# shaunplee/ray-tracing

Hardware: AMD Instinct MI355X
Metric: Msamples/s (WxHxspp/s) + achieved HBM GB/s, final scene 1200x800x500spp (higher is better)
Workload: dtype f64

## Files before the change

include/rt_wide.h:

```cpp
#pragma once
#include <stdint.h>

#define RT_WIDE 4

typedef struct rt_wnode {
  float lo[3][RT_WIDE];
  float hi[3][RT_WIDE];
  int32_t child[RT_WIDE];
  int32_t pad[RT_WIDE];
} rt_wnode;

typedef struct rt_qnode {
  float origin[3];
  float scale[3];
  uint32_t qlo[3];
  uint32_t qhi[3];
  int32_t child[RT_WIDE];
} rt_qnode;

#define RT_WKEY_BITS 14
#define RT_WKEY_MASK ((1u << RT_WKEY_BITS) - 1u)
#define RT_WKEY_MAX_IDS (1 << (RT_WKEY_BITS - 1))
#define RT_WKEY_REJECTED 0x7f800000u

#if defined(__HIPCC__) || defined(__CUDACC__)
#define RT_WKEY_FN __host__ __device__ static inline
#else
#define RT_WKEY_FN static inline
#endif

RT_WKEY_FN int rt_wkey_fits(long long n_wide_nodes, long long n_leaf_slots) {
  return n_wide_nodes <= RT_WKEY_MAX_IDS && n_leaf_slots <= RT_WKEY_MAX_IDS;
}
RT_WKEY_FN int32_t rt_wkey_pack(uint32_t key_bits, int32_t ref) {
  return (int32_t)((key_bits & ~RT_WKEY_MASK) | ((uint32_t)ref & RT_WKEY_MASK));
}
RT_WKEY_FN int32_t rt_wkey_ref(int32_t word) {
  const uint32_t low = (uint32_t)word & RT_WKEY_MASK;
  return (int32_t)(low ^ (1u << (RT_WKEY_BITS - 1))) - (1 << (RT_WKEY_BITS - 1));
}

RT_WKEY_FN int rt_wkey_beyond(int32_t word, float tmax32, float slack) {
  const uint32_t kb = (uint32_t)word & ~RT_WKEY_MASK;
  float key;
  __builtin_memcpy(&key, &kb, sizeof key);
  return key * (1.0f - 0x1p-21f) > __builtin_fmaf(tmax32, 1.0f + 0x1p-21f, slack);
}

#ifdef __cplusplus
static_assert(sizeof(rt_wnode) == 128, "rt_wnode is 128 bytes");
static_assert(sizeof(rt_qnode) == 64, "rt_qnode is 64 bytes");
#endif
```

ray-tracing_amd/csrc/rt_kernels.h:

```cpp
#pragma once
#include <hip/hip_runtime.h>

#include <algorithm>
#include <cstdlib>
#include <cmath>
#include <cstdio>
#include <cstring>
#include <string>
#include <vector>

#include "rt.h"
#include "rt_device.h"
#include "rt_error.h"
#include "rt_internal.h"
#include "rt_trace.h"

using namespace rtd;

namespace {

struct UDiv {
  uint32_t m;
  int s1, s2;
};
// ... 259 lines not shown
        } else {
          w = -1;
        }
      }
    }
    if (w < 0) break;
    if (!path) {
      const uint32_t pid = (uint32_t)((long long)row * L.W + px);
      g.init(A.seed, pid, (uint32_t)s);
      g.reserve(3);
      const double ru = g.draw(), rv = g.draw();
      const int y = L.H - 1 - row;
      const double u = ((double)px + ru) / (double)L.W;
      const double v = ((double)y + rv) / (double)L.H;
      ray = get_ray(L.cam, u, v, g);
      thr = v3(1.0, 1.0, 1.0);
      depth = L.max_depth;
      path = true;
    }
    V3 contrib;
    if constexpr ((F & F_COUNT) != 0) {
      segs += depth > 0;
      s1 = stamp();
      s2 = s1;
    }
    bool ended = segment<F>(A, S, L.S, ray, thr, depth, g, stk, contrib, cnt, stride, &s2);
    if (!ended && thr.x != thr.x && thr.y != thr.y && thr.z != thr.z) {
      contrib = vmul(thr, v3(0.0, 0.0, 0.0));
      ended = true;
    }
    if constexpr ((F & F_COUNT) != 0) {
      const unsigned long long s3 = stamp();
      ph_acq += s1 - s0;
      ph_trav += s2 - s1;
      ph_shade += s3 - s2;
    }
    if (ended) {
      if constexpr ((F & F_COUNT) != 0) {
        blocks += g.pair;
        ++samples;
      }
      if (A.flags & RT_FLAG_NAN_ZERO) contrib = nan_zero(contrib);
      sum = sum + contrib;
      path = false;
      ++s;
      const bool all_nan = (A.flags & RT_FLAG_NAN_CULL) && sum.x != sum.x && sum.y != sum.y && sum.z != sum.z;
      if (s == s_end || all_nan) {
        store_partial(L, w, sum);
        w = -1;
      }
    }
  }
  if constexpr ((F & F_COUNT) != 0) {
    wave_add(&L.work[0], segs);
    wave_add(&L.work[1], cnt.box);
    wave_add(&L.work[2], cnt.prim);
    wave_add(&L.work[3], cnt.other);
    wave_add(&L.work[4], cnt.light);
    wave_add(&L.work[5], blocks);
    wave_add(&L.work[6], samples);
    if ((threadIdx.x & 63) == 0) {
      atomicAdd(&L.work[8], ph_acq);
      atomicAdd(&L.work[9], ph_trav);
      atomicAdd(&L.work[10], ph_shade);
    }
  }
}

template <unsigned F, int WAVES>
__global__ void __launch_bounds__(RT_BLOCK, WAVES) render_philox(RenderArgs A) {
  __shared__ __attribute__((aligned(16))) int stk_mem[kLcBytes / 4 + RT_STACK * RT_BLOCK];
  const LaunchConst& L = stage_const(A, stk_mem);
  __syncthreads();
  philox_loop<F>(A, L, A.S, &stk_mem[kLcBytes / 4 + threadIdx.x], RT_BLOCK);
}

template <unsigned F, int WAVES>
__global__ void __launch_bounds__(WAVES * 256, WAVES) render_philox_lds(RenderArgs A, int n_nodes, int stack_entries) {
  extern __shared__ __attribute__((aligned(16))) unsigned char lds[];
  const LaunchConst& L = stage_const(A, lds);
  rt_node* nodes = reinterpret_cast<rt_node*>(lds + kLcBytes);
  {
    const uint4* src = reinterpret_cast<const uint4*>(A.S.nodes);
    uint4* dst = reinterpret_cast<uint4*>(lds + kLcBytes);
    const int n16 = n_nodes * (int)(sizeof(rt_node) / 16);
    for (int i = threadIdx.x; i < n16; i += blockDim.x) dst[i] = src[i];
  }
  __syncthreads();
  Scene S = A.S;
  S.nodes = nodes;
  int* stk = reinterpret_cast<int*>(lds + kLcBytes + (size_t)n_nodes * sizeof(rt_node)) + threadIdx.x;
  (void)stack_entries;
  philox_loop<F>(A, L, S, stk, WAVES * 256);
}


template <unsigned F, bool PK = false>
__device__ __forceinline__ void philox_loop2(const RenderArgs& A, const LaunchConst& L, const Scene& S, int* stk,
                                             int stride, int* side_p, volatile uint32_t* wq) {
  const int lane = threadIdx.x & 63;
  const unsigned long long lanes_below = (lane == 0) ? 0ull : (~0ull >> (64 - lane));
  const bool joint = !(A.flags & RT_FLAG_REFERENCE_CULL);

  long long w = -1;
  bool done = false, walking = false, ready = false;
  if (lane == 0) {
    wq[0] = 0u;
    wq[1] = 0u;
  }
  constexpr int kLoop = (F & F_WIDE) ? 2 : 1;
  constexpr bool kLaneLds = lane_lds_of(F, kLoop);
  int l_px = 0, l_row = 0, l_s_end = 0, l_depth = 0;
  int* ex = side_p + side_ints_of(F, S.frames, kLoop) * stride;
  int& px = kLaneLds ? ex[0] : l_px;
  int& row = kLaneLds ? ex[stride] : l_row;
  int& s_end = kLaneLds ? ex[2 * stride] : l_s_end;
  int& depth = kLaneLds ? ex[3 * stride] : l_depth;
  px = 0, row = 0, s_end = 0, depth = 0;
  int s = 0;
  V3 thr = v3(0, 0, 0), sum = v3(0, 0, 0);
  RngPhilox g;
  g.init(A.seed, 0, 0);
  Trav t;
  Side side{side_p, stride, S.frames};
  Cnt cnt{};
  if constexpr ((F & F_COUNT) != 0) cnt.prof = A.prof;
  unsigned long long segs = 0, blocks = 0, samples = 0, ph_setup = 0, ph_trav = 0, ph_shade = 0;

  auto end_sample = [&](V3 contrib) __attribute__((always_inline)) {
    if constexpr ((F & F_COUNT) != 0) {
      blocks += g.pair;
      ++samples;
    }
    if (A.flags & RT_FLAG_NAN_ZERO) contrib = nan_zero(contrib);
    const V3 sm = sum + contrib;
    sum = sm;
    ++s;
    const bool all_nan = (A.flags & RT_FLAG_NAN_CULL) && sm.x != sm.x && sm.y != sm.y && sm.z != sm.z;
    if (s == s_end || all_nan) {
      if (kTail<F> && w >= kTailSlot) store_partial_at(L.tail_buf, w - kTailSlot, contrib);
      else store_partial(L, w, sm);
      w = -1;
    }
  };
  auto all_nan3 = [](const V3& a) __attribute__((always_inline)) { return a.x != a.x && a.y != a.y && a.z != a.z; };

  for (;;) {
    unsigned long long s0 = 0;
    if constexpr ((F & F_COUNT) != 0) {
      s0 = stamp();
      ++cnt.oslot;
    }
    if (ready && (t.tie || (kRefMixed<F> && t.lite)) && !t.redo) {
      ready = false;
      if constexpr ((F & F_COUNT) != 0) ++cnt.ties;
      trav_redo<F>(t, L.S.world_ref, INFINITY);
      if constexpr ((F & F_WIDE) != 0) t.ray = prep(plain(t.ray));
      walking = true;
    }
    bool start = false;
    if (ready) {
      ready = false;
      Hit h;
      Ray ray = plain(t.ray);
      const bool got = trav_finish<F>(L.S, t, ray, kEps, h, side);
      V3 contrib;
      V3 th = thr;
      if (shade_hit<F>(L.S, got, h, ray, th, depth, g, contrib, cnt)) {
        end_sample(contrib);
      } else if (depth <= 0 || all_nan3(th)) {
        end_sample(vmul(th, v3(0.0, 0.0, 0.0)));
      } else {
        thr = th;
        t.ray.o = ray.o;
        t.ray.d = ray.d;
        t.ray.tm = ray.tm;
        start = true;
        if constexpr ((F & F_COUNT) != 0) ++segs;
      }
    }
    unsigned long long s0b = 0;
    if constexpr ((F & F_COUNT) != 0) s0b = stamp();
    while (!walking && !start) {
      for (;;) {
        const bool need = (w < 0) && !done;
        const unsigned long long mask = __ballot(need);
        if (!mask) break;
        const uint32_t n_need = (uint32_t)__popcll(mask);
        const uint32_t q_next = wq[0], q_end = wq[1];
        const uint32_t avail = q_end - q_next;
        uint32_t base2 = q_next, end2 = q_end;
        if (avail < n_need) {
          const int leader = __ffsll((long long)mask) - 1;
          unsigned long long claim = 0;
          if (lane == leader) {
            const uint32_t want = n_need - avail;
            const long long rem = L.work_total - (long long)q_end;
            const uint32_t b = rem <= 0 ? 0u : max((uint32_t)L.batch_floor,
                                                   (uint32_t)fminf((float)L.batch, (float)rem * L.batch_per_item));
            const uint32_t got = want < b ? b : want;
            const unsigned long long c0 = atomicAdd(L.counter, (unsigned long long)got);
            claim = (c0 < 0xffff0000ull ? c0 : 0xffff0000ull) | ((unsigned long long)got << 32);
          }
          const unsigned long long c1 = __shfl(claim, leader);
          base2 = (uint32_t)c1;
          end2 = base2 + (uint32_t)(c1 >> 32);
        }
        const uint32_t rank = (uint32_t)__popcll(mask & lanes_below);
        if (need) {
          const long long wi = (long long)(rank < avail ? q_next + rank : base2 + (rank - avail));
          if (wi >= L.work_total) {
            done = true;
          } else if (kTail<F> ? work_unit<(F & F_SKIP) != 0>(L, (uint32_t)wi, px, row, s, s_end, w)
                              : work_item<(F & F_SKIP) != 0>(L, (uint32_t)wi, px, row, s, s_end, w)) {
            sum = v3(0, 0, 0);
          } else {
            w = -1;
          }
        }
        const int leader = __ffsll((long long)mask) - 1;
        if (lane == leader) {
          wq[0] = avail < n_need ? base2 + (n_need - avail) : q_next + n_need;
          wq[1] = end2;
        }
      }
      if (w < 0) break;
      const uint32_t pid = (uint32_t)((long long)row * L.W + px);
      g.init(A.seed, pid, (uint32_t)s);
      g.reserve(3);
      const double ru = g.draw(), rv = g.draw();
      const int y = L.H - 1 - row;
      const double u = ((double)px + ru) / (double)L.W;
      const double v = ((double)y + rv) / (double)L.H;
      const Ray cray = get_ray(L.cam, u, v, g);
      t.ray.o = cray.o;
      t.ray.d = cray.d;
      t.ray.tm = cray.tm;
      thr = v3(1.0, 1.0, 1.0);
      depth = L.max_depth;
      if (depth <= 0) {
        end_sample(vmul(v3(1.0, 1.0, 1.0), v3(0.0, 0.0, 0.0)));
        continue;
      }
      start = true;
      if constexpr ((F & F_COUNT) != 0) ++segs;
    }
    if (start) {
      trav_begin<F>(t, plain(t.ray), S.world, kEps, INFINITY);
      if (S.ref_walk) trav_restart_ref(t, S.world, INFINITY);
      trav_media_first<F>(S, t, kEps, cnt, g, side);
      walking = true;
    }
    if (!walking) break;
    unsigned long long s1 = 0;
    if constexpr ((F & F_COUNT) != 0) s1 = stamp();
    const int live = __popcll(__ballot(true));
    const int stop = (live * A.trav_stop) >> 6;
    const int ls = (F & F_WIDE) ? A.leaf_stop : A.box_first;
    walk_until<F, PK>(S, t, walking, kEps, stk, stride, joint, stop, (live * ls) >> 6, cnt, g, side, A.med_batch);
    ready = !walking;
    if constexpr ((F & F_COUNT) != 0) {
      const unsigned long long s2 = stamp();
      ph_shade += s0b - s0;
      ph_setup += s1 - s0b;
      ph_trav += s2 - s1;
    }
  }
  if constexpr ((F & F_COUNT) != 0) {
    wave_add(&L.work[0], segs);
    wave_add(&L.work[1], cnt.box);
    wave_add(&L.work[2], cnt.prim);
    wave_add(&L.work[3], cnt.other);
    wave_add(&L.work[4], cnt.light);
    wave_add(&L.work[5], blocks);
    wave_add(&L.work[6], samples);
    wave_add(&L.work[7], cnt.wide);
    wave_add(&L.work[11], cnt.islot);
    wave_add(&L.work[12], cnt.lslot);
    wave_add(&L.work[13], cnt.oslot);
    wave_add(&L.work[14], cnt.phit);
    wave_add(&L.work[15], cnt.ties);
    if ((threadIdx.x & 63) == 0) {
      atomicAdd(&L.work[8], ph_setup);
      atomicAdd(&L.work[9], ph_trav);
      atomicAdd(&L.work[10], ph_shade);
    }
  }
}

template <unsigned F>
constexpr int lane_ints() {
  return ((F & (F_WIDE | F_MIXW)) ? RT_WSTACK : RT_STACK) + ((F & F_FRAMES) ? kSideInts : 0);
}

template <unsigned F, int WAVES>
__global__ void __launch_bounds__(RT_BLOCK, WAVES) render_philox2(RenderArgs A, int stack_entries) {
  extern __shared__ __attribute__((aligned(16))) int stk_mem[];
  __shared__ uint32_t wave_q[RT_BLOCK / 64][2];
  const LaunchConst& L = stage_const(A, stk_mem);
  __syncthreads();
  int* lane0 = &stk_mem[kLcBytes / 4 + threadIdx.x];
  philox_loop2<F>(A, L, A.S, lane0, RT_BLOCK, lane0 + stack_entries * RT_BLOCK,
                  wave_q[__builtin_amdgcn_readfirstlane(threadIdx.x >> 6)]);
}

template <unsigned F>
__global__ void __launch_bounds__(RT_BLOCK, 1) render_philox2_count_packed(RenderArgs A, int stack_entries) {
  static_assert((F & F_WIDE) != 0 && (F & F_COUNT) != 0, "the 4-wide counting build only");
  extern __shared__ __attribute__((aligned(16))) int stk_mem[];
  __shared__ uint32_t wave_q[RT_BLOCK / 64][2];
  const LaunchConst& L = stage_const(A, stk_mem);
// ... 757 lines not shown
```

ray-tracing_amd/csrc/rt_trace.h:

```cpp
#pragma once
#include "rt_device.h"

namespace rtd {

template <unsigned F>
constexpr bool kRay32 = (F & (F_WIDE | F_MIXW)) != 0;
template <unsigned F>
constexpr bool kNoInv = (F & F_WIDE) != 0 && (F & (F_ALL | F_MIXW)) == 0;

struct Cnt {
  unsigned box, prim, other, light, wide;
  unsigned islot, lslot, oslot;
  unsigned phit;
  unsigned ties;
  unsigned long long* prof;
};
enum : unsigned { K_BOX = 1u, K_WIDE = 2u, K_LEAF = 4u, K_MEDIUM = 8u, K_FRAME = 16u };

__device__ __forceinline__ int hmod256(long long a) {
  const long long r = a % 256;
  return (int)(r < 0 ? r + 256 : r);
}
__device__ inline double noise(const rt_perlin* P, double sc, V3 p) {
  const V3 q = scale(sc, p);
// ... 804 lines not shown
  }
  if constexpr ((F & F_MEDIA) != 0) {
    const Ray r = plain(t.ray);
    const double rec1tp = gmax(t_min, t1);
    const double rec2t = R::kKeyed ? tt : gmin(t.closest, tt);
    if (rec1tp >= rec2t) return;
    const double rec1t = rec1tp < 0 ? 0 : rec1tp;
    const double ray_length = vlen(r.d);
    const double dist_inside = (rec2t - rec1t) * ray_length;
    double rnd;
    if constexpr (R::kKeyed) rnd = g.keyed(medium_key(n));
    else rnd = g.draw();
    const double hit_dist = n->f[0] * log_call(rnd);
    if (hit_dist > dist_inside) return;
    const double x = rec1t + (hit_dist / ray_length);
    if constexpr (R::kKeyed) {
      if (!(x <= t.closest)) return;
      trav_take<F>(S, t, x, id, kSubMedium, side, refsem, n, false);
    } else {
      trav_take<F>(S, t, x, id, kSubMedium, side, true, n, false);
    }
  }
}

typedef float f32x2 __attribute__((ext_vector_type(2)));

__device__ __forceinline__ void wide_keys2(const Trav& t, f32x2 nx, f32x2 ny, f32x2 nz, f32x2 fx, f32x2 fy, f32x2 fz,
                                           float& k0, float& k1) {
  const f32x2 ox = {t.o32x, t.o32x}, oy = {t.o32y, t.o32y}, oz = {t.o32z, t.o32z};
  const f32x2 ix = {t.i32x, t.i32x}, iy = {t.i32y, t.i32y}, iz = {t.i32z, t.i32z};
  const f32x2 tnx = (nx - ox) * ix, tny = (ny - oy) * iy, tnz = (nz - oz) * iz;
  const f32x2 tfx = (fx - ox) * ix, tfy = (fy - oy) * iy, tfz = (fz - oz) * iz;
  const float n0 = fmaxf(fmaxf(tnx.x, tny.x), fmaxf(tnz.x, t.tmin32));
  const float n1 = fmaxf(fmaxf(tnx.y, tny.y), fmaxf(tnz.y, t.tmin32));
  const float f0 = fminf(fminf(tfx.x, tfy.x), fminf(tfz.x, t.tmax32));
  const float f1 = fminf(fminf(tfx.y, tfy.y), fminf(tfz.y, t.tmax32));
  const bool h0 = n0 * (1.0f - 0x1p-21f) <= fmaf(f0, 1.0f + 0x1p-21f, t.slack);
  const bool h1 = n1 * (1.0f - 0x1p-21f) <= fmaf(f1, 1.0f + 0x1p-21f, t.slack);
  k0 = h0 ? fminf(n0, 3.0e38f) : INFINITY;
  k1 = h1 ? fminf(n1, 3.0e38f) : INFINITY;
}

__device__ __forceinline__ void cswap(float& ka, int& ca, float& kb, int& cb) {
  const bool s = kb < ka;
  const float k = s ? kb : ka;
  const int c = s ? cb : ca;
  kb = s ? ka : kb;
  cb = s ? ca : cb;
  ka = k;
  ca = c;
}

__device__ __forceinline__ void pswap(int& a, int& b) {
  const int lo = min(a, b);
  b = max(a, b);
  a = lo;
}

__device__ __forceinline__ float4 qplanes(uint32_t q, float s, float o) {
  return float4{fmaf((float)(q & 255u), s, o), fmaf((float)((q >> 8) & 255u), s, o),
                fmaf((float)((q >> 16) & 255u), s, o), fmaf((float)(q >> 24), s, o)};
}

template <unsigned F = 0, bool PK = false>
__device__ __forceinline__ bool wide_node(const Scene& S, Trav& t, int* stk, int stride, int w) {
  float4 nx, ny, nz, fx, fy, fz;
  int4 ch;
  if constexpr ((F & F_QNODE) != 0) {
    const uint4* qb = reinterpret_cast<const uint4*>(&S.qnodes[w]);
    const uint4 a = qb[0], b = qb[1], c = qb[2];
    const uint4 d = qb[3];
    ch = int4{(int)d.x, (int)d.y, (int)d.z, (int)d.w};
    const float ox = __uint_as_float(a.x), oy = __uint_as_float(a.y), oz = __uint_as_float(a.z);
    const float sx = __uint_as_float(a.w), sy = __uint_as_float(b.x), sz = __uint_as_float(b.y);
    const bool mx = signbit(t.i32x), my = signbit(t.i32y), mz = signbit(t.i32z);
    nx = qplanes(mx ? c.y : b.z, sx, ox);
    fx = qplanes(mx ? b.z : c.y, sx, ox);
    ny = qplanes(my ? c.z : b.w, sy, oy);
    fy = qplanes(my ? b.w : c.z, sy, oy);
    nz = qplanes(mz ? c.w : c.x, sz, oz);
    fz = qplanes(mz ? c.x : c.w, sz, oz);
  } else {
    const float* base = reinterpret_cast<const float*>(&S.wnodes[w]);
    const int ox = signbit(t.i32x) ? 12 : 0, oy = signbit(t.i32y) ? 16 : 4, oz = signbit(t.i32z) ? 20 : 8;
    nx = *reinterpret_cast<const float4*>(base + ox);
    ny = *reinterpret_cast<const float4*>(base + oy);
    nz = *reinterpret_cast<const float4*>(base + oz);
    fx = *reinterpret_cast<const float4*>(base + (ox ^ 12));
    fy = *reinterpret_cast<const float4*>(base + (oy < 12 ? oy + 12 : oy - 12));
    fz = *reinterpret_cast<const float4*>(base + (oz < 12 ? oz + 12 : oz - 12));
    ch = *reinterpret_cast<const int4*>(base + 24);
  }
  float k0, k1, k2, k3;
  wide_keys2(t, f32x2{nx.x, nx.y}, f32x2{ny.x, ny.y}, f32x2{nz.x, nz.y}, f32x2{fx.x, fx.y}, f32x2{fy.x, fy.y},
             f32x2{fz.x, fz.y}, k0, k1);
  wide_keys2(t, f32x2{nx.z, nx.w}, f32x2{ny.z, ny.w}, f32x2{nz.z, nz.w}, f32x2{fx.z, fx.w}, f32x2{fy.z, fy.w},
             f32x2{fz.z, fz.w}, k2, k3);
  int c0 = ch.x, c1 = ch.y, c2 = ch.z, c3 = ch.w;
  const int n_hit = (k0 < INFINITY) + (k1 < INFINITY) + (k2 < INFINITY) + (k3 < INFINITY);
  if constexpr (PK) {
    int p0 = rt_wkey_pack(__float_as_uint(k0), c0), p1 = rt_wkey_pack(__float_as_uint(k1), c1);
    int p2 = rt_wkey_pack(__float_as_uint(k2), c2), p3 = rt_wkey_pack(__float_as_uint(k3), c3);
    pswap(p0, p1);
    pswap(p2, p3);
    pswap(p0, p2);
    pswap(p1, p3);
    pswap(p1, p2);
    c0 = rt_wkey_ref(p0);
    c1 = p1;
    c2 = p2;
    c3 = p3;
  } else {
    cswap(k0, c0, k1, c1);
    cswap(k2, c2, k3, c3);
    cswap(k0, c0, k2, c2);
    cswap(k1, c1, k3, c3);
    cswap(k1, c1, k2, c2);
  }
  const int e0 = n_hit > 3 ? c3 : (n_hit > 2 ? c2 : c1);
  const int e1 = n_hit > 3 ? c2 : c1;
  stk[t.sp * stride] = e0;
  stk[(t.sp + 1) * stride] = e1;
  stk[(t.sp + 2) * stride] = c1;
  t.sp += n_hit > 1 ? n_hit - 1 : 0;
  t.node = c0;
  return n_hit != 0;
}

constexpr int kNone = (int)0x80000000;

template <unsigned F>
__device__ __forceinline__ bool trav_pop_mixed(const Scene& S, Trav& t, const int* stk, int stride, Side& side,
                                               double t_min = kEps) {
  bool reb = false;
  for (;;) {
    const bool end = t.sp == 0;
    const int e = end ? 0 : stk[(--t.sp) * stride];
    const bool frame = (F & F_FRAMES) && ((F & F_MIXW) ? (e >= 0 && (e & RT_FRAME)) : (e & RT_FRAME));
    if (end || !frame) {
      if ((F & F_FRAMES) && reb) {
        Ray pr = side.get_ray();
        for (int k = 0; k < t.level; ++k) pr = enter_instance(&S.nodes[side.frame(k)], pr);
        t.ray = prep(pr);
        if constexpr ((F & F_MIXW) != 0) set_ray32(t, t_min);
      }
      t.node = e;
      return !end;
    }
    --t.level;
    reb = true;
  }
}

template <unsigned F, class R>
__device__ __forceinline__ bool trav_step(const Scene& S, Trav& t, double t_min, int* stk, int stride, bool joint,
                                          Cnt& cnt, R& g, Side& side) {
  bool wide = false;
  if constexpr ((F & F_WIDE) != 0) wide = !t.ref;
  if (wide) {
    if (t.node >= 0) {
      if constexpr ((F & F_COUNT) != 0) ++cnt.wide;
      if (wide_node<F>(S, t, stk, stride, t.node)) return true;
    } else {
      const rt_node* n = &S.leaves[~t.node];
      trav_leaf<F>(S, t, n, ~t.node | kSlotTag, t_min, cnt, g, side, false);
    }
    if (t.sp == 0) return false;
    t.node = stk[(--t.sp) * stride];
    return true;
  }
  bool leaf_slot = false, to_wide = false;
  if constexpr ((F & F_MIXW) != 0) {
    to_wide = t.node >= 0 && (t.node & RT_WNODE);
    leaf_slot = t.node < 0;
  }
  if (!to_wide) {
  int id = leaf_slot ? (~(t.node | RT_ISMED) | kSlotTag) : (t.node & ~(RT_SUB | RT_IDTAGS));
  int tag = leaf_slot ? RT_SUB : (kRefMixed<F> ? (t.node & RT_SUB) : 0);
  bool refsem = t.ref && !tag;
  const rt_node* n = leaf_slot ? &S.leaves[~(t.node | RT_ISMED)] : &S.nodes[id];
  const int tf = n->type;
  const int type = tf & RT_TYPE_MASK;
  if (type == RT_NODE_BVH) {
   constexpr int kFuse = (F & F_WIDE) ? 0 : 8;
   for (int fuse = 0;; ++fuse) {
    if (fuse) {
      id = t.node & ~(RT_SUB | RT_IDTAGS);
      tag = kRefMixed<F> ? (t.node & RT_SUB) : 0;
      refsem = t.ref && !tag;
      n = &S.nodes[id];
    }
    const bool same = kRefMixed<F> && (t.node & RT_IDTAGS) == RT_SAMEBOX;
    if constexpr ((F & F_COUNT) != 0) cnt.box += !same;
    if (same || box_hit(n->f, t.ray, t_min, refsem ? t.closest : closest_up<F>(t), joint)) {
      const int c = n->c;
      const bool ord = (c & RT_BVH_ORDERED) && !t.redo;
      if constexpr ((F & F_MIXW) != 0) {
        if (ord && (c & RT_WROOT)) {
          t.node = RT_WNODE | ((c >> 2) & RT_WROOT_MASK);
          to_wide = true;
          break;
        }
      }
      const bool flip = ord && !(c & RT_BVH_MEDIA_FIRST) && comp(t.ray.d, c & 3) < 0;
      const int ctag = (kRefMixed<F> && ord) ? RT_SUB : tag;
      stk[(t.sp++) * stride] = (flip ? n->a : n->b) | ctag;
      t.node = (flip ? n->b : n->a) | ctag;
      if ((t.node & RT_ISBOX) && fuse < kFuse) continue;
      return true;
    }
    break;
   }
  } else if ((F & F_FRAMES) && (type == RT_NODE_TRANSLATE || type == RT_NODE_ROTATE) && !(tf & RT_CHAIN_PRIM)) {
    if (t.level == 0) side.put_ray(plain(t.ray));
    Ray cr = plain(t.ray);
    int cur = leaf_slot ? n->c : id, ct = tf;
    if ((F & F_MIXW) && leaf_slot && (tf & RT_FRAME_FUSED)) {
      rt_node rec;
      {
        const uint4* q = reinterpret_cast<const uint4*>(n);
        const uint4 q0 = q[0], q1 = q[1], q2 = q[2], q3 = q[3];
        uint4* r = reinterpret_cast<uint4*>(&rec);
        r[0] = q0, r[1] = q1, r[2] = q2, r[3] = q3;
      }
      cur = rec.c;
      if constexpr ((F & F_COUNT) != 0) ++cnt.other;
      side.frame(t.level++) = cur;
      stk[(t.sp++) * stride] = RT_FRAME | cur;
      cr = enter_instance(&rec, cr);
      if (tf & RT_FRAME_FUSED2) {
        if constexpr ((F & F_COUNT) != 0) ++cnt.other;
        side.frame(t.level++) = rec.a;
        stk[(t.sp++) * stride] = RT_FRAME | rec.a;
        const int ax = (tf >> RT_FRAME_AX2_SHIFT) & 3;
        cr = Ray{unrotate_point(ax, rec.f[3], rec.f[4], cr.o), unrotate_point(ax, rec.f[3], rec.f[4], cr.d), cr.tm};
      }
      const int inner = (int)rec.f[5];
      t.ray = prep(cr);
      set_ray32(t, t_min);
      t.node = (inner & RT_WNODE) ? inner : (inner | tag);
      return true;
    } else {
      do {
        if constexpr ((F & F_COUNT) != 0) ++cnt.other;
        side.frame(t.level++) = cur;
        stk[(t.sp++) * stride] = RT_FRAME | cur;
        cr = enter_instance(&S.nodes[cur], cr);
        cur = S.nodes[cur].a;
        ct = S.nodes[cur].type;
      } while (((ct & RT_TYPE_MASK) == RT_NODE_TRANSLATE || (ct & RT_TYPE_MASK) == RT_NODE_ROTATE) &&
               !(ct & RT_CHAIN_PRIM));
    }
    t.ray = prep(cr);
    if constexpr ((F & F_MIXW) != 0) set_ray32(t, t_min);
    t.node = cur | tag;
    return true;
  } else {
    trav_leaf<F>(S, t, n, id, t_min, cnt, g, side, refsem);
  }
  if (!to_wide) return trav_pop_mixed<F>(S, t, stk, stride, side, t_min);
  }
  if constexpr ((F & F_MIXW) != 0) {
    if constexpr ((F & F_COUNT) != 0) ++cnt.wide;
    refresh_ray32(t);
    if (wide_node<F>(S, t, stk, stride, t.node & ~RT_WNODE)) return true;
  }
  return trav_pop_mixed<F>(S, t, stk, stride, side, kEps);
}


template <bool PK = false>
__device__ __forceinline__ int trav_pop(Trav& t, const int* stk, int stride) {
  if constexpr (PK) {
    return t.sp ? rt_wkey_ref(stk[(--t.sp) * stride]) : kNone;
  } else {
    return t.sp ? stk[(--t.sp) * stride] : kNone;
  }
}
template <bool PK = false>
__device__ __forceinline__ void trav_postpone(Trav& t, int* stk, int stride) {
  if (t.node < 0 && t.node != kNone && t.pend < 0) {
    t.pend = ~t.node;
    t.node = trav_pop<PK>(t, stk, stride);
  }
}
template <unsigned F, bool PK = false>
__device__ __forceinline__ void wide_inner(const Scene& S, Trav& t, int* stk, int stride, Cnt& cnt) {
  if constexpr ((F & F_COUNT) != 0) ++cnt.wide;
  if (!wide_node<F, PK>(S, t, stk, stride, t.node)) t.node = trav_pop<PK>(t, stk, stride);
  trav_postpone<PK>(t, stk, stride);
}
template <unsigned F, bool PK = false, class R>
__device__ __forceinline__ void wide_leaf(const Scene& S, Trav& t, double t_min, int* stk, int stride, Cnt& cnt, R& g,
                                          Side& side) {
  for (int k = 0; k < 1 && t.pend >= 0; ++k) {
    const rt_node* n = &S.leaves[t.pend];
    [[maybe_unused]] const float bound_before = t.tmax32;
    trav_leaf<F>(S, t, n, t.pend | kSlotTag, t_min, cnt, g, side, false);
    t.pend = -1;
    if constexpr (PK && (F & F_RECT) == 0) {
      if (t.tmax32 < bound_before)
        while (t.sp && rt_wkey_beyond(stk[(t.sp - 1) * stride], t.tmax32, t.slack)) --t.sp;
    }
  }
  trav_postpone<PK>(t, stk, stride);
}

template <unsigned F, bool PK = false, class R>
__device__ __forceinline__ void walk_until(const Scene& S, Trav& t, bool& walking, double t_min, int* stk, int stride,
                                           bool joint, int stop, int leaf_stop, Cnt& cnt, R& g, Side& side,
                                           int med_batch = 0) {
  if constexpr ((F & F_WIDE) == 0) {
    for (;;) {
      const int n_walk = __popcll(__ballot(walking));
      if (n_walk <= stop) break;
      constexpr bool kBoxFirst = kRefMixed<F>;
      const bool box_id = walking && t.node >= 0 && (t.node & (RT_ISBOX | RT_WNODE));
      const bool at_box = kBoxFirst && box_id;
      int ty = -1;
      if constexpr ((F & F_COUNT) != 0) {
        if (walking) {
          if ((F & F_MIXW) && t.node < 0) ty = S.leaves[~(t.node | RT_ISMED)].type & RT_TYPE_MASK;
          else if (box_id) ty = RT_NODE_BVH;
          else ty = S.nodes[t.node & ~(RT_SUB | RT_IDTAGS)].type & RT_TYPE_MASK;
        }
      }
      bool go = walking;
      if constexpr (kBoxFirst) {
        const int n_box = __popcll(__ballot(at_box));
        if (leaf_stop < n_walk && n_box > leaf_stop) {
          go = walking && at_box;
        } else if ((F & F_MEDIA) && med_batch > 0) {
          const bool at_med = walking && t.node >= 0 && (t.node & (RT_WNODE | RT_IDTAGS)) == RT_ISMED;
          const int n_med = __popcll(__ballot(at_med));
          if (n_med < med_batch && n_med < n_walk) go = walking && !at_med;
        }
      }
      if constexpr ((F & F_COUNT) != 0) {
        ++cnt.islot;
        const bool inst = ty == RT_NODE_TRANSLATE || ty == RT_NODE_ROTATE;
        const bool box = ty == RT_NODE_BVH;
        cnt.lslot += (__ballot(go && box) != 0) + (__ballot(go && inst) != 0) +
                     (__ballot(go && ty == RT_NODE_CONSTANT_MEDIUM) != 0) +
                     (__ballot(go && !box && !inst && ty != RT_NODE_CONSTANT_MEDIUM) != 0);
      }
      unsigned kinds = 0;
      unsigned long long t0 = 0;
      if constexpr ((F & F_COUNT) != 0) {
        const bool wide = walking && t.node >= 0 && (t.node & RT_WNODE);
        const bool inst = ty == RT_NODE_TRANSLATE || ty == RT_NODE_ROTATE;
        bool frame = false;
        if (inst) {
          const int nid = t.node < 0 ? -1 : (t.node & ~(RT_SUB | RT_IDTAGS));
          const int tf = t.node < 0 ? S.leaves[~(t.node | RT_ISMED)].type : S.nodes[nid].type;
          frame = !(tf & RT_CHAIN_PRIM);
        }
        kinds = (__ballot(go && ty == RT_NODE_BVH && !wide) ? K_BOX : 0u) | (__ballot(go && wide) ? K_WIDE : 0u) |
                (__ballot(go && ty == RT_NODE_CONSTANT_MEDIUM) ? K_MEDIUM : 0u) | (__ballot(go && frame) ? K_FRAME : 0u) |
                (__ballot(go && ty >= 0 && ty != RT_NODE_BVH && ty != RT_NODE_CONSTANT_MEDIUM && !frame) ? K_LEAF : 0u);
        t0 = stamp();
      }
      if (go) walking = trav_step<F>(S, t, t_min, stk, stride, joint, cnt, g, side);
      if constexpr ((F & F_COUNT) != 0) {
        const unsigned long long t1 = stamp();
        if (cnt.prof && __lane_id() == (unsigned)(__ffsll((long long)__ballot(true)) - 1)) {
          atomicAdd(&cnt.prof[kinds], t1 - t0);
          atomicAdd(&cnt.prof[32 + kinds], 1ull);
        }
      }
    }
  } else {
    for (;;) {
      if (__popcll(__ballot(walking)) <= stop) break;
      const bool seeking = walking && (t.ref || (t.pend < 0 && t.node >= 0));
      const bool holding = walking && !t.ref && t.pend >= 0;
      unsigned kinds = 0;
      unsigned long long t0 = 0;
      if constexpr ((F & F_COUNT) != 0) t0 = stamp();
      if (__popcll(__ballot(seeking)) > leaf_stop || __ballot(holding) == 0) {
        if constexpr ((F & F_COUNT) != 0) {
          ++cnt.islot;
          kinds = __ballot(walking && t.ref) ? K_BOX | K_WIDE : K_WIDE;
        }
        if (walking && t.ref) {
          walking = trav_step<F>(S, t, t_min, stk, stride, joint, cnt, g, side);
        } else if (walking && t.node >= 0) {
          wide_inner<F, PK>(S, t, stk, stride, cnt);
          walking = t.node != kNone || t.pend >= 0;
        }
      } else {
        if constexpr ((F & F_COUNT) != 0) {
          ++cnt.lslot;
          kinds = K_LEAF;
        }
        if (holding) {
          wide_leaf<F, PK>(S, t, t_min, stk, stride, cnt, g, side);
          walking = t.node != kNone || t.pend >= 0;
        }
      }
      if constexpr ((F & F_COUNT) != 0) {
        const unsigned long long t1 = stamp();
        if (cnt.prof && __lane_id() == (unsigned)(__ffsll((long long)__ballot(true)) - 1)) {
          atomicAdd(&cnt.prof[kinds], t1 - t0);
          atomicAdd(&cnt.prof[32 + kinds], 1ull);
        }
      }
    }
  }
}

template <unsigned F>
__device__ __forceinline__ bool trav_finish(const Scene& S, const Trav& t, const Ray& r, double t_min, Hit& h,
                                            const Side& side) {
  if (t.best_node < 0) return false;
  const bool slot = (F & (F_WIDE | F_MIXW)) && (t.best_node & kSlotTag);
  const rt_node* n = slot ? &S.leaves[t.best_node & ~kSlotTag] : &S.nodes[t.best_node];
  int levels = 0;
  if constexpr ((F & F_FRAMES) != 0) levels = t.best_level;
  Ray fr = r;
  int sub = t.best_sub;
  const rt_node* leaf = n;
  int chain_id = -1, chain_len = 0;
  if constexpr ((F & F_FRAMES) != 0)
    for (int k = 0; k < levels; ++k) fr = enter_instance(&S.nodes[side.best(k)], fr);
  bool med = false;
  if constexpr ((F & F_MEDIA) != 0) med = sub == kSubMedium;
  if (med) {
    h.t = t.closest;
    h.p = at(fr, t.closest);
    h.n = v3(1, 0, 0);
    h.u = 0;
    h.v = 0;
    h.ff = 1;
    h.mat = n->b;
  }
  if constexpr ((F & F_INST) != 0) {
    if (!med && (sub & kSubChain)) {
      sub &= ~kSubChain;
      chain_id = slot ? n->c : t.best_node;
      int cur = chain_id;
      while ((S.nodes[cur].type & RT_TYPE_MASK) == RT_NODE_TRANSLATE || (S.nodes[cur].type & RT_TYPE_MASK) == RT_NODE_ROTATE) {
        fr = enter_instance(&S.nodes[cur], fr);
        cur = S.nodes[cur].a;
        ++chain_len;
      }
      leaf = &S.nodes[cur];
    }
  }
  if (!med) prim_record<F>(S, leaf, sub, fr, t.closest, h);
  for (int lv = levels + chain_len - 1; lv >= 0; --lv) {
    Ray rl = r;
    const rt_node* inst = nullptr;
    int cur = chain_id;
    for (int k = 0; k <= lv; ++k) {
      if ((F & F_FRAMES) && k < levels) {
        inst = &S.nodes[side.best(k)];
      } else {
        inst = &S.nodes[cur];
        cur = inst->a;
      }
      rl = enter_instance(inst, rl);
    }
    exit_instance(inst, rl, h);
  }
  return true;
}

template <unsigned F, int D>
__device__ __forceinline__ double htbl_pdf_value(const Scene& S, int id, V3 origin, V3 v, const RayX& r) {
  id &= ~RT_IDTAGS;
  const rt_node* n = &S.nodes[id];
  const int type = n->type & RT_TYPE_MASK;
  Hit hh;
  if (type == RT_NODE_RECT_XZ) {
    if (!rect_hit(1, n->f[0], n->f[1], n->f[2], n->f[3], n->f[4], n->a, r, kEps, INFINITY, hh)) return 0.0;
    const double area = (n->f[1] - n->f[0]) * (n->f[3] - n->f[2]);
    const double distance_squared = hh.t * hh.t * sqlen(v);
    const double cosine = fabs(dot(v, hh.n) / vlen(v));
    return distance_squared / (cosine * area);
  }
  if (type == RT_NODE_SPHERE) {
    double t;
    if (!sphere_t(vload(n->f), n->f[3], r, kEps, INFINITY, t)) return 0.0;
    const double radius = n->f[3];
    const double cos_theta_max = sqrt(1 - radius * radius / sqlen(vload(n->f) - origin));
    const double solid_angle = 2 * kPi * (1 - cos_theta_max);
    return 1 / solid_angle;
  }
  if constexpr (D > 0) {
    if (type == RT_NODE_BVH) {
      if (!box_hit(n->f, r, kEps, INFINITY, false)) return 0.0;
      const double left_pdf = htbl_pdf_value<F, D - 1>(S, n->a, origin, v, r) + 0;
      const double left_w = (double)S.nodes[n->a & ~RT_IDTAGS].c / (double)n->c;
      const double right_pdf = htbl_pdf_value<F, D - 1>(S, n->b, origin, v, r) + 0;
      const double right_w = (double)S.nodes[n->b & ~RT_IDTAGS].c / (double)n->c;
      return left_w * left_pdf + right_w * right_pdf;
    }
  }
  return 0.0;
}

template <class R>
__device__ inline V3 htbl_random(const Scene& S, int id, V3 o, R& g) {
  if (id >= 0) id &= ~RT_IDTAGS;
  while (id >= 0 && (S.nodes[id].type & RT_TYPE_MASK) == RT_NODE_BVH) {
    const rt_node* n = &S.nodes[id];
    const double rd = g.draw();
    id = (rd < (double)S.nodes[n->a & ~RT_IDTAGS].c / (double)n->c ? n->a : n->b) & ~RT_IDTAGS;
  }
  if (id < 0) return v3(1, 0, 0);
  const rt_node* n = &S.nodes[id];
  const int type = n->type & RT_TYPE_MASK;
  if (type == RT_NODE_RECT_XZ) {
    const double rx = draw_r(g, n->f[0], n->f[1]);
    const double rz = draw_r(g, n->f[2], n->f[3]);
    return v3(rx, n->f[4], rz) - o;
  }
  if (type == RT_NODE_SPHERE) {
    const V3 dir = vload(n->f) - o;
    const double dist_squared = sqlen(dir);
    const ONB uvw = onb_from_w(dir);
    const V3 rts = random_to_sphere(g, n->f[3], dist_squared);
    return onb_local(uvw, rts);
// ... 108 lines not shown
```

Baseline: 5298.

## Add lean wide-BVH walk loop that resolves ties inline and drops ref-path branching

For packed-key wide traversal without rect primitives, adds a specialized walk loop whose lane state (walking, seeking, holding) is derived from node, pend and stack pointer instead of a separate walking flag and ref-mode branches. Tie and lite redo rays are now fully re-traversed inline in a per-lane loop through the non-wide path, rather than being fed back into the cooperative walk. Stack culling and postponement are rewritten as branch-light selects. The aim is fewer divergent branches and less state in the hot wide loop, at the cost of serialized per-lane redo work when ties occur.

```diff
diff --git a/include/rt_wide.h b/include/rt_wide.h
--- a/include/rt_wide.h
+++ b/include/rt_wide.h
@@ -47,6 +47,28 @@
   return key * (1.0f - 0x1p-21f) > __builtin_fmaf(tmax32, 1.0f + 0x1p-21f, slack);
 }
 
+#define RT_WNONE ((int32_t)0x80000000)
+
+RT_WKEY_FN int rt_wlane_walking(int32_t node, int32_t pend) { return (node != RT_WNONE) | (pend >= 0); }
+RT_WKEY_FN int rt_wlane_seeking(int32_t node, int32_t pend) { return (pend < 0) & (node >= 0); }
+RT_WKEY_FN int rt_wlane_holding(int32_t pend) { return pend >= 0; }
+
+typedef struct rt_wstep {
+  int32_t node, pend, sp;
+} rt_wstep;
+
+RT_WKEY_FN int32_t rt_wstep_slot(int32_t sp) { return sp > 0 ? sp - 1 : 0; }
+
+RT_WKEY_FN rt_wstep rt_wstep_postpone(int32_t node, int32_t pend, int32_t sp, int32_t word) {
+  const int park = (node < 0) & (node != RT_WNONE) & (pend < 0);
+  const int has = sp > 0;
+  rt_wstep s;
+  s.node = park ? (has ? rt_wkey_ref(word) : RT_WNONE) : node;
+  s.pend = park ? ~node : pend;
+  s.sp = sp - (park & has);
+  return s;
+}
+
 #ifdef __cplusplus
 static_assert(sizeof(rt_wnode) == 128, "rt_wnode is 128 bytes");
 static_assert(sizeof(rt_qnode) == 64, "rt_qnode is 64 bytes");
diff --git a/ray-tracing_amd/csrc/rt_kernels.h b/ray-tracing_amd/csrc/rt_kernels.h
--- a/ray-tracing_amd/csrc/rt_kernels.h
+++ b/ray-tracing_amd/csrc/rt_kernels.h
@@ -435,11 +435,17 @@
       ++cnt.oslot;
     }
     if (ready && (t.tie || (kRefMixed<F> && t.lite)) && !t.redo) {
-      ready = false;
       if constexpr ((F & F_COUNT) != 0) ++cnt.ties;
       trav_redo<F>(t, L.S.world_ref, INFINITY);
       if constexpr ((F & F_WIDE) != 0) t.ray = prep(plain(t.ray));
-      walking = true;
+      if constexpr (kLeanWalk<F, PK>) {
+        while (trav_step<F, true>(S, t, kEps, stk, stride, joint, cnt, g, side)) {
+        }
+        t.node = kNone;
+      } else {
+        ready = false;
+        walking = true;
+      }
     }
     bool start = false;
     if (ready) {
diff --git a/ray-tracing_amd/csrc/rt_trace.h b/ray-tracing_amd/csrc/rt_trace.h
--- a/ray-tracing_amd/csrc/rt_trace.h
+++ b/ray-tracing_amd/csrc/rt_trace.h
@@ -980,11 +980,11 @@
   }
 }
 
-template <unsigned F, class R>
+template <unsigned F, bool REDO = false, class R>
 __device__ __forceinline__ bool trav_step(const Scene& S, Trav& t, double t_min, int* stk, int stride, bool joint,
                                           Cnt& cnt, R& g, Side& side) {
   bool wide = false;
-  if constexpr ((F & F_WIDE) != 0) wide = !t.ref;
+  if constexpr ((F & F_WIDE) != 0 && !REDO) wide = !t.ref;
   if (wide) {
     if (t.node >= 0) {
       if constexpr ((F & F_COUNT) != 0) ++cnt.wide;
@@ -1112,6 +1112,10 @@
     t.node = trav_pop<PK>(t, stk, stride);
   }
 }
+static_assert(RT_WNONE == kNone, "rt_wide.h's end-of-walk node is Trav's");
+template <unsigned F, bool PK>
+constexpr bool kLeanWalk = PK && (F & F_WIDE) != 0 && (F & F_RECT) == 0;
+
 template <unsigned F, bool PK = false>
 __device__ __forceinline__ void wide_inner(const Scene& S, Trav& t, int* stk, int stride, Cnt& cnt) {
   if constexpr ((F & F_COUNT) != 0) ++cnt.wide;
@@ -1127,11 +1131,24 @@
     trav_leaf<F>(S, t, n, t.pend | kSlotTag, t_min, cnt, g, side, false);
     t.pend = -1;
     if constexpr (PK && (F & F_RECT) == 0) {
-      if (t.tmax32 < bound_before)
-        while (t.sp && rt_wkey_beyond(stk[(t.sp - 1) * stride], t.tmax32, t.slack)) --t.sp;
-    }
-  }
-  trav_postpone<PK>(t, stk, stride);
+      if (t.tmax32 < bound_before) {
+        for (;;) {
+          const int top = rt_wstep_slot(t.sp);
+          const int word = stk[top * stride];
+          if (!((t.sp > 0) & (rt_wkey_beyond(word, t.tmax32, t.slack) != 0))) break;
+          t.sp = top;
+        }
+      }
+    }
+  }
+  if constexpr (kLeanWalk<F, PK>) {
+    const rt_wstep s = rt_wstep_postpone(t.node, t.pend, t.sp, stk[rt_wstep_slot(t.sp) * stride]);
+    t.node = s.node;
+    t.pend = s.pend;
+    t.sp = s.sp;
+  } else {
+    trav_postpone<PK>(t, stk, stride);
+  }
 }
 
 template <unsigned F, bool PK = false, class R>
@@ -1197,6 +1214,35 @@
         }
       }
     }
+  } else if constexpr (kLeanWalk<F, PK>) {
+    for (;;) {
+      if (__popcll(__ballot(rt_wlane_walking(t.node, t.pend))) <= stop) break;
+      unsigned kinds = 0;
+      unsigned long long t0 = 0;
+      if constexpr ((F & F_COUNT) != 0) t0 = stamp();
+      if (__popcll(__ballot(rt_wlane_seeking(t.node, t.pend))) > leaf_stop ||
+          __ballot(rt_wlane_holding(t.pend)) == 0) {
+        if constexpr ((F & F_COUNT) != 0) {
+          ++cnt.islot;
+          kinds = K_WIDE;
+        }
+        if (t.node >= 0) wide_inner<F, PK>(S, t, stk, stride, cnt);
+      } else {
+        if constexpr ((F & F_COUNT) != 0) {
+          ++cnt.lslot;
+          kinds = K_LEAF;
+        }
+        if (rt_wlane_holding(t.pend)) wide_leaf<F, PK>(S, t, t_min, stk, stride, cnt, g, side);
+      }
+      if constexpr ((F & F_COUNT) != 0) {
+        const unsigned long long t1 = stamp();
+        if (cnt.prof && __lane_id() == (unsigned)(__ffsll((long long)__ballot(true)) - 1)) {
+          atomicAdd(&cnt.prof[kinds], t1 - t0);
+          atomicAdd(&cnt.prof[32 + kinds], 1ull);
+        }
+      }
+    }
+    walking = rt_wlane_walking(t.node, t.pend);
   } else {
     for (;;) {
       if (__popcll(__ballot(walking)) <= stop) break;
```

After: 5615 (median of 6 runs). 1.06x the previous value.
